# Fanchuana/OPUS-PLLM

Measured on AMD Instinct MI355X. Metric: proteins_per_sec, higher is better.
Workload: dtype f16; 1 GPU; OPUS-PLLM-llama3_8b shape: batch 64/GPU, 512-residue proteins, 89-id prompt (+8 protein tokens = 96 positions), 32 new tokens, greedy (BASELINE configs[3] per-GPU shard: batch 512 over 8 GPUs); batch_per_gpu=64, residues=512, parallelism=replicas x1 (batch-sharded), all-gather of ids

## Files before the change

### include/opus_pllm.h

```cpp
#ifndef OPUS_PLLM_H
#define OPUS_PLLM_H

#include <stdint.h>

#ifdef __cplusplus
extern "C" {
#endif

#define OPUS_ABI_VERSION 10

enum opus_status {
    OPUS_OK = 0,
    OPUS_EBADARG = -1,
    OPUS_ESHAPE = -2,
    OPUS_EHIP = -3,
    OPUS_ERCCL = -4,
    OPUS_EUNSUPPORTED = -5,
    OPUS_ESTATE = -6
};

enum opus_dtype { OPUS_F16 = 0, OPUS_F32 = 1, OPUS_I32 = 2, OPUS_I64 = 3, OPUS_U8 = 4, OPUS_F8E4M3 = 5, OPUS_I8 = 6,
                  OPUS_F4E2M1X2 = 7, OPUS_E8M0 = 8 };

typedef struct opus_config {
// ... 160 lines not shown
int opus_debug_argmax_lse(opus_ctx *ctx, const float *d_logits, int32_t B, int32_t V, int32_t *d_idx, float *d_lse, void *stream);
int opus_debug_guidance(opus_ctx *ctx, float *d_logits, int32_t P, int32_t V, float guidance_scale, void *stream);

int opus_set_logits_processors(opus_ctx *ctx, float repetition_penalty, int32_t no_repeat_ngram_size, int32_t min_new_tokens,
                               const int32_t *bad_ids, const int32_t *bad_offsets, int32_t n_bad);
int opus_debug_logits_process(opus_ctx *ctx, float *d_logits, int32_t B, int32_t V, const int32_t *d_hist, int32_t hist_stride,
                              int32_t hist_len, const int32_t *eos_ids, int32_t n_eos, float repetition_penalty,
                              int32_t no_repeat_ngram_size, int32_t min_new_tokens, const int32_t *bad_ids,
                              const int32_t *bad_offsets, int32_t n_bad, void *stream);

int opus_set_token_constraint(opus_ctx *ctx, int32_t n_states, const int32_t *edge_off, const int32_t *edge_tok,
                              const int32_t *edge_next, int32_t n_edges, const uint8_t *completing, const int32_t *end_ids,
                              int32_t n_end, const int32_t *start, int32_t n_start, void *stream);
int opus_debug_token_constraint(opus_ctx *ctx, float *d_logits, int32_t B, int32_t V, const int32_t *d_hist, int32_t hist_stride,
                                int32_t hist_len, int32_t *d_state_out, void *stream);

int opus_debug_gemm(opus_ctx *ctx, const void *d_A, const void *d_W, const float *d_bias, const float *d_residual,
                    void *d_C, int32_t M, int32_t N, int32_t K, int32_t epi, int32_t out_f32, void *stream);
int opus_debug_gemm_norm(opus_ctx *ctx, const float *d_A, const void *d_W, void *d_C, int32_t M, int32_t N, int32_t K,
                         int32_t epi, int32_t out_f32, float eps, void *stream);
int opus_debug_gemm_slabs(opus_ctx *ctx, const void *d_A, const void *d_W, float *d_slabs, int32_t M, int32_t N, int32_t K,
                          int32_t *ks, void *stream);
int opus_debug_gemm_plan(opus_ctx *ctx, int32_t *plan);
int opus_debug_gemm_w8(opus_ctx *ctx, int32_t form, const void *d_A, const void *d_W, const void *d_q8, const void *d_e8,
                       const float *d_bias, const float *d_residual, void *d_C, int32_t M, int32_t N, int32_t K, int32_t epi,
                       int32_t out_f32, float eps, int32_t *ks, int32_t *ran_w8, void *stream);
int opus_debug_gemm_w4(opus_ctx *ctx, int32_t form, const void *d_A, const void *d_W, const void *d_q4, const void *d_s4,
                       const float *d_bias, const float *d_residual, void *d_C, int32_t M, int32_t N, int32_t K, int32_t epi,
                       int32_t out_f32, float eps, int32_t *ks, int32_t *ran_w4, void *stream);
int opus_debug_knob(opus_ctx *ctx, const char *name, int32_t value);
int opus_debug_gemm_rowscale(opus_ctx *ctx, const void *d_A, const void *d_W1, float *d_X, const void *d_W2, void *d_C,
                             int32_t M, int32_t N1, int32_t K1, int32_t N2, int32_t epi, float eps, int32_t *fused,
                             void *stream);
int opus_debug_gemm_rope(opus_ctx *ctx, const void *d_A, const void *d_W, const float *d_bias, void *d_out, int32_t M,
                         int32_t D, int32_t K, int32_t T, int32_t heads, int32_t allow_fuse, int32_t *fused, void *stream);
int opus_debug_gemm_ln(opus_ctx *ctx, const void *d_A, const void *d_W1, const float *d_b1, float *d_X, float *d_part, void *d_xh,
                       float *d_stat, const void *d_W2, const float *d_c2, const float *d_colsum, void *d_C, int32_t M, int32_t N1,
                       int32_t K1, int32_t N2, int32_t epi, int32_t rms, float eps, int32_t rope_T, const int32_t *d_rope_pos,
                       int32_t *produced, int32_t *plan, void *stream);
int opus_debug_attention(opus_ctx *ctx, const void *d_Q, const void *d_K, const void *d_V, void *d_O,
                         const int32_t *d_kstart, const int32_t *d_kend, int32_t B, int32_t T, int32_t heads,
                         int32_t group, int32_t head_dim, int32_t causal, float scale, void *stream);

int opus_debug_attn_prefill(opus_ctx *ctx, const void *d_Q, const void *d_K, const void *d_V, void *d_O, int64_t q_st, int64_t k_st,
                            int64_t v_st, int64_t o_st, int64_t q_sb, int64_t k_sb, int64_t v_sb, int64_t o_sb,
                            const int32_t *d_kstart, const int32_t *d_kend, const int32_t *d_cu, int32_t B, int32_t T,
                            int32_t heads, int32_t group, int32_t head_dim, int32_t causal, int32_t q_trim, float scale,
                            int32_t *qt_used, void *stream);

int opus_debug_attn_decode(opus_ctx *ctx, const void *d_qkv, const void *d_k_hist, const void *d_v_hist, const int32_t *d_kstart,
                           int32_t B, int32_t T0, int32_t step, void *d_out, void *d_k_new, void *d_v_new, void *stream);

int opus_debug_attn_decode_form(opus_ctx *ctx, const void *d_qkv, const float *d_slabs, int32_t ks, const float *d_row_ssq,
                                int32_t row_nblk, int32_t K, float eps, const float *d_bias, const void *d_k_hist,
                                const void *d_v_hist, const int32_t *d_kstart, int32_t B, int32_t T0, int32_t step,
                                int32_t out_tiled, void *d_out, void *d_k_new, void *d_v_new, void *d_k_cache, void *d_v_cache,
                                int32_t *gp_used, void *stream);

int opus_check_error(opus_ctx *ctx, void *stream);

int opus_beam_topk(opus_ctx *ctx, const float *d_run_scores, int32_t B, int32_t K, int32_t M, float *d_scores, int32_t *d_idx,
                   void *stream);
int opus_kv_reorder(opus_ctx *ctx, const int32_t *d_src_rows, int32_t R, void *stream);
int opus_beam_sample_topk(opus_ctx *ctx, const float *d_logits, const float *d_run_scores, int32_t B, int32_t K, int32_t M,
                          float temperature, float top_p, uint64_t seed, int32_t step, float *d_scores, int32_t *d_idx, void *stream);
int opus_set_sampling_top_k(opus_ctx *ctx, int32_t k);
// ... 27 lines not shown
```

### opus-pllm_amd/_cabi.py

```python
from __future__ import annotations

import ctypes as C
import os
from typing import Optional

from .config import OpusConfig

_HERE = os.path.dirname(os.path.abspath(__file__))
BF16 = os.environ.get("OPUS_DTYPE", "fp16").lower() in ("bf16", "bfloat16")
LIB_PATH = os.environ.get("OPUS_LIB_PATH") or os.path.join(_HERE, "lib", "libopus_pllm_bf16.so" if BF16 else "libopus_pllm.so")
ABI_VERSION = 10

OPUS_F16, OPUS_F32, OPUS_I32, OPUS_I64, OPUS_U8 = 0, 1, 2, 3, 4
OPUS_F8E4M3, OPUS_I8 = 5, 6
OPUS_F4E2M1X2, OPUS_E8M0 = 7, 8


def operand_dtype():
    import torch
    return torch.bfloat16 if BF16 else torch.float16


class OpusError(RuntimeError):
    def __init__(self, code: int, msg: str):
# ... 123 lines not shown
    "opus_llama_score_tree": (C.c_int, [_P, _P, C.c_int32, _P, _P, _P, C.c_int32, _P, C.c_int32, _P, _P, _P, C.c_int32, _P, _P, _P,
                                        C.c_int32, _P, C.c_int32, _P, _P, C.c_int32, C.c_int64, _P, _P, C.c_int64, _P, C.c_int64, _P]),
    "opus_llama_score_tree_scratch_bytes": (C.c_int64, [C.POINTER(CConfig), C.c_int32, C.c_int32, C.c_int32, C.c_int32, C.c_int32,
                                                        C.c_int32]),
    "opus_llama_dec_rows_cap": (C.c_int64, [C.POINTER(CConfig)]),
    "opus_llama_tree_max_depth": (C.c_int32, []),
    "opus_trie_path_sums": (C.c_int, [_P, _P, _P, _P, _P, _P, C.c_int32, C.c_int32, C.c_int32, _P, _P]),
    "opus_debug_attn_tree": (C.c_int, [_P, _P, _P, _P, _P, C.c_int32, C.c_int32, C.c_int32, _P, _P, _P, _P, _P]),
    "opus_debug_xent": (C.c_int, [_P, _P, C.c_int32, C.c_int32, _P, _P, _P, _P]),
    "opus_esm2_contacts_packed": (C.c_int, [_P, _P, C.POINTER(C.c_int32), C.c_int32, _P, _P, _P, C.c_int64, _P]),
    "opus_esm2_contacts_scratch_bytes": (C.c_int64, [C.POINTER(CConfig), C.POINTER(C.c_int32), C.c_int32]),
    "opus_debug_contacts": (C.c_int, [_P, _P, _P, C.c_int64, C.POINTER(C.c_int32), C.c_int32, C.c_int32, C.c_int32, _P, _P, _P, _P,
                                      _P, C.c_int64, _P]),
    "opus_esm2_lm_head": (C.c_int, [_P, _P, C.c_int32, C.c_int32, _P, _P]),
    "opus_debug_esm2_lm_head": (C.c_int, [_P, _P, C.c_int32, C.c_int32, _P, _P]),
    "opus_generate_scored": (C.c_int, [_P, _P, _P, C.c_int32, C.c_int32, C.c_int32, C.POINTER(C.c_int32), C.c_int32, C.c_int32,
                                       C.c_float, C.c_float, C.c_uint64, _P, C.POINTER(C.c_int32), _P, _P, _P, _P]),
    "opus_llama_prefill_fanout": (C.c_int, [_P, _P, _P, C.c_int32, C.c_int32, C.c_int32, _P, _P]),
    "opus_generate_scored_fanout": (C.c_int, [_P, _P, _P, C.c_int32, C.c_int32, C.c_int32, C.c_int32, C.POINTER(C.c_int32), C.c_int32,
                                              C.c_int32, C.c_float, C.c_float, C.c_uint64, _P, C.POINTER(C.c_int32), _P, _P, _P, _P]),
    "opus_debug_argmax_lse": (C.c_int, [_P, _P, C.c_int32, C.c_int32, _P, _P, _P]),
    "opus_generate_scored_guided": (C.c_int, [_P, _P, _P, C.c_int32, C.c_int32, C.c_float, C.c_int32, C.POINTER(C.c_int32), C.c_int32,
                                              C.c_int32, C.c_float, C.c_float, C.c_uint64, _P, C.POINTER(C.c_int32), _P, _P, _P, _P]),
    "opus_debug_guidance": (C.c_int, [_P, _P, C.c_int32, C.c_int32, C.c_float, _P]),
    "opus_set_logits_processors": (C.c_int, [_P, C.c_float, C.c_int32, C.c_int32, C.POINTER(C.c_int32), C.POINTER(C.c_int32),
                                             C.c_int32]),
    "opus_debug_logits_process": (C.c_int, [_P, _P, C.c_int32, C.c_int32, _P, C.c_int32, C.c_int32, C.POINTER(C.c_int32), C.c_int32,
                                            C.c_float, C.c_int32, C.c_int32, C.POINTER(C.c_int32), C.POINTER(C.c_int32), C.c_int32,
                                            _P]),
    "opus_set_token_constraint": (C.c_int, [_P, C.c_int32, _P, _P, _P, C.c_int32, _P, _P, C.c_int32, _P, C.c_int32, _P]),
    "opus_debug_token_constraint": (C.c_int, [_P, _P, C.c_int32, C.c_int32, _P, C.c_int32, C.c_int32, _P, _P]),
    "opus_debug_gemm_rowscale": (C.c_int, [_P, _P, _P, _P, _P, _P, C.c_int32, C.c_int32, C.c_int32, C.c_int32, C.c_int32,
                                           C.c_float, C.POINTER(C.c_int32), _P]),
    "opus_debug_gemm_ln": (C.c_int, [_P, _P, _P, _P, _P, _P, _P, _P, _P, _P, _P, _P, C.c_int32, C.c_int32, C.c_int32, C.c_int32,
                                     C.c_int32, C.c_int32, C.c_float, C.c_int32, _P, C.POINTER(C.c_int32), C.POINTER(C.c_int32), _P]),
}

_lib: Optional[C.CDLL] = None


def lib() -> C.CDLL:
    global _lib
    if _lib is not None:
        return _lib
    if not os.path.exists(LIB_PATH):
        raise OpusError(-100, f"{LIB_PATH} not found: build it with `python opus-pllm_amd/build.py` "
                              "(hipcc --offload-arch=gfx950); this package has no CPU fallback")
    l = C.CDLL(LIB_PATH)
    for name, (res, args) in SIGNATURES.items():
        fn = getattr(l, name)
        fn.restype = res
        fn.argtypes = args
    v = l.opus_abi_version()
    if v != ABI_VERSION:
        raise OpusError(-101, f"ABI version mismatch: library {v}, binding {ABI_VERSION}")
    if l.opus_operand_dtype() != (1 if BF16 else 0):
        raise OpusError(-102, f"{LIB_PATH} was not built for {'bf16' if BF16 else 'fp16'} operands")
    _lib = l
    return l


def check(code: int) -> None:
    if code != 0:
        raise OpusError(code, lib().opus_last_error().decode("utf-8", "replace"))
```

### opus-pllm_amd/csrc/api.cpp

```cpp
#include "../../include/opus_pllm.h"
#include "common.h"

#include <cmath>
#include <cstdarg>
#include <cstdio>
#include <cstdlib>
#include <cstring>
#include <algorithm>
#include <atomic>
#include <map>
#include <string>
#include <vector>

using namespace opus;

static thread_local char g_err[512] = "";
static int fail(int code, const char *fmt, ...) {
    va_list ap;
    va_start(ap, fmt);
    vsnprintf(g_err, sizeof(g_err), fmt, ap);
    va_end(ap);
    return code;
}
#define HIPC(expr)                                                                                   \
// ... 3181 lines not shown
    const int hd = D / heads;
    if (hd != c->cfg.enc_dim / c->cfg.enc_heads || T > c->cfg.max_enc_tokens)
        return fail(OPUS_ESHAPE, "debug_gemm_rope: head_dim / T must match the context's encoder rotary table");
    HIPC(hipSetDevice(c->device));
    hipStream_t s = (hipStream_t)stream;
    const float qs = 1.0f / sqrtf((float)hd);
    GemmGot got;
    OPC(gemm(c, s, (const half_t *)A, K, (const half_t *)W, M, 3 * D, K, bias, EPI_NONE, nullptr, out, 3 * D, 0,
             GemmAsk().rope(allow_fuse && hd == 64 ? c->cs_enc : nullptr, nullptr, T, D, qs), &got));
    *fused = got.rope_done;
    if (!got.rope_done) HIPC(launch_esm_rope((half_t *)out, c->cs_enc, M / T, T, heads, hd, qs, s));
    return OPUS_OK;
}

extern "C" int opus_debug_gemm_rowscale(opus_ctx *c, const void *A, const void *W1, float *X, const void *W2, void *Cp, int32_t M,
                                        int32_t N1, int32_t K1, int32_t N2, int32_t epi, float eps, int32_t *fused, void *stream) {
    if (!c || !A || !W1 || !X || !W2 || !Cp || !fused) return fail(OPUS_EBADARG, "debug_gemm_rowscale: null pointer");
    if (M < 1 || N1 < 64 || N1 % 64 || K1 < 64 || K1 % 64 || N2 < 32) return fail(OPUS_ESHAPE, "debug_gemm_rowscale: shape");
    if (epi != EPI_NONE && epi != EPI_SILU_GU16) return fail(OPUS_EBADARG, "debug_gemm_rowscale: epilogue 0 or 2");
    const opus_config &g = c->cfg;
    if ((int64_t)M * N1 > (int64_t)g.max_batch * g.max_prompt * g.dec_dim) return fail(OPUS_ESHAPE, "debug_gemm_rowscale: M * N1 exceeds the scratch");
    HIPC(hipSetDevice(c->device));
    hipStream_t s = (hipStream_t)stream;
    ResidShadow sh;
    GemmGot got;
    OPC(gemm(c, s, (const half_t *)A, K1, (const half_t *)W1, M, N1, K1, nullptr, EPI_NONE, X, X, N1, 1,
             GemmAsk().copy16(fuse_rows() && M <= 96 ? c->d_xn : nullptr), &got));
    sh.produced(X, got);
    *fused = sh.xh_src != nullptr && (N1 & 255) == 0 && gemm_goes_wide(M, N2) ? 1 : 0;
    const int nout = epi == EPI_SILU_GU16 ? N2 / 2 : N2;
    return gemm_norm(c, s, sh, X, eps, c->d_xn, (const half_t *)W2, M, N2, N1, epi, Cp, nout, 0);
}

extern "C" int opus_debug_gemm_ln(opus_ctx *c, const void *A, const void *W1, const float *b1, float *X, float *part, void *xh,
                                  float *stat, const void *W2, const float *c2, const float *colsum, void *Cp, int32_t M, int32_t N1,
                                  int32_t K1, int32_t N2, int32_t epi, int32_t rms, float eps, int32_t rope_T,
                                  const int32_t *rope_pos, int32_t *produced, int32_t *plan, void *stream) {
    if (!c || !A || !W1 || !X || !part || !xh || !stat || !W2 || !Cp || !produced || !plan)
        return fail(OPUS_EBADARG, "debug_gemm_ln: null pointer");
    if (M < 1 || N1 < 64 || N1 % 64 || K1 < 64 || K1 % 64 || N2 < 32) return fail(OPUS_ESHAPE, "debug_gemm_ln: shape");
    if (epi != EPI_NONE && epi != EPI_GELU && epi != EPI_SILU_GU16) return fail(OPUS_EBADARG, "debug_gemm_ln: epilogue 0, 1 or 2");
    if (epi == EPI_SILU_GU16 && (!rms || c2 || colsum || N2 % 32))
        return fail(OPUS_EBADARG, "debug_gemm_ln: the gate / up epilogue is the RMSNorm form (no bias, no column sums)");
    if (rms ? colsum != nullptr : colsum == nullptr) return fail(OPUS_EBADARG, "debug_gemm_ln: column sums go with LayerNorm only");
    if (rope_pos && rope_T < 1) return fail(OPUS_EBADARG, "debug_gemm_ln: rope_pos needs rope_T");
    if (rope_T > 0 && (epi != EPI_NONE || N2 % 3 || (N2 / 3) % 64 || c->cfg.enc_dim / c->cfg.enc_heads != 64 ||
                       rope_T > c->cfg.max_enc_tokens))
        return fail(OPUS_ESHAPE, "debug_gemm_ln: rotary needs EPI_NONE, N2 = 3 D, head_dim 64 and rope_T within the context's table");
    HIPC(hipSetDevice(c->device));
    hipStream_t s = (hipStream_t)stream;
    c->phase = PH_OTHER;
    for (int i = 0; i < 2 * PP_PLAN_WORDS; ++i) plan[i] = -1;
    HIPC(hipMemsetAsync(c->d_cnt, 0, HANDOFF_ERR * sizeof(int32_t), s));
    GemmGot got;
    OPC(gemm(c, s, (const half_t *)A, K1, (const half_t *)W1, M, N1, K1, b1, EPI_NONE, X, X, N1, 1,
             GemmAsk().ln_produce(gemm_goes_pp(M, N1) ? part : nullptr, (half_t *)xh).report_pp(plan), &got));
    *produced = got.ln_done;
    if (!got.ln_done) return OPUS_OK;
    KL(KC_NORM, 8.0 * M * (N1 / 64), launch_ln_finalize(part, M, N1 / 64, N1, eps, rms, stat, s));
    const int nout = epi == EPI_SILU_GU16 ? N2 / 2 : N2;
    OPC(gemm(c, s, (const half_t *)xh, N1, (const half_t *)W2, M, N2, N1, c2, epi, nullptr, Cp, nout, 0,
             GemmAsk().ln_consume(stat, colsum).report_pp(plan + PP_PLAN_WORDS)
                 .rope(rope_T > 0 ? c->cs_enc : nullptr, rope_pos, rope_T, N2 / 3, 0.125f), &got));
    if (rope_T > 0 && !got.rope_done) return fail(OPUS_ESTATE, "debug_gemm_ln: the consumer GEMM did not fuse the rotary");
    return OPUS_OK;
}
// ... 375 lines not shown
```

### opus-pllm_amd/csrc/common.h

```cpp
#pragma once
#include <hip/hip_runtime.h>
#include <hip/hip_ext.h>
#include <stdint.h>

namespace opus {

#ifdef OPUS_BF16
typedef __bf16 half_t;
typedef __bf16 h8 __attribute__((ext_vector_type(8)));
typedef __bf16 h4 __attribute__((ext_vector_type(4)));
typedef __bf16 h2 __attribute__((ext_vector_type(2)));
#else
typedef _Float16 half_t;
typedef _Float16 h8 __attribute__((ext_vector_type(8)));
typedef _Float16 h4 __attribute__((ext_vector_type(4)));
typedef _Float16 h2 __attribute__((ext_vector_type(2)));
#endif
typedef float f4 __attribute__((ext_vector_type(4)));
__device__ __forceinline__ f4 mfma16(h8 a, h8 b, f4 c) {
#ifdef OPUS_BF16
    return __builtin_amdgcn_mfma_f32_16x16x32_bf16(a, b, c, 0, 0, 0);
#else
    return __builtin_amdgcn_mfma_f32_16x16x32_f16(a, b, c, 0, 0, 0);
#endif
// ... 116 lines not shown
    const float *bias;
    const float *residual;
    int64_t ldr;
    void *C;
    int64_t ldc;
    int out_f32;
    int epi;
    float *ws;
    int64_t ws_bytes;
    half_t *xh_out;
    float *ssq_out;
    int *fused_done;
    const float *row_ssq;
    int row_nblk;
    int64_t ssq_cap = 0;
    int *nblk_out = nullptr;
    int slab_only = 0;
    int *ks_out = nullptr;
    int force_wide = 0;
    const float *rope_cs = nullptr;
    const int32_t *rope_pos = nullptr;
    int rope_T = 0, rope_cols = 0, rope_qcols = 0;
    float rope_qscale = 1.0f;
    int *rope_done = nullptr;
    int a_tiled = 0, xh_tiled = 0, c_tiled = 0;
    int *combine_cnt = nullptr;
    float *ln_part = nullptr;
    int *ln_done = nullptr;
    const float *ln_stat = nullptr;
    const float *ln_colsum = nullptr;
    int pp_gm = 8;
    int stagger = 0;
    int no_rot = 0;
    long long *trace = nullptr;
    int *pp_plan = nullptr;
    int *plan = nullptr;
    const uint8_t *q8 = nullptr;
    const int8_t *e8 = nullptr;
    int *ran_w8 = nullptr;
    const uint8_t *q4 = nullptr;
    const uint8_t *s4 = nullptr;
    int *ran_w4 = nullptr;
};
constexpr int PP_PLAN_WORDS = 5;
enum PpTail { PP_TAIL_NONE = 0, PP_TAIL_PAIR = 1, PP_TAIL_REDUCE = 2 };
constexpr int GEMM_PLAN_WORDS = 8;
enum GemmCombine { GC_NONE = 0, GC_REDUCE = 1, GC_REDUCE4 = 2, GC_IN_LAUNCH = 3, GC_PP_PAIR = 4, GC_PP_REDUCE = 5, GC_SLABS = 6 };
inline void gemm_plan_set(const GemmParams &p, int klass, int mt, int tn, int ns, int alds, int P, int ks, int combine) {
    if (!p.plan) return;
    const int v[GEMM_PLAN_WORDS] = {klass, mt, tn, ns, alds, P, ks, combine};
    for (int i = 0; i < GEMM_PLAN_WORDS; ++i) p.plan[i] = v[i];
}

struct AttnParams {
    const half_t *Q, *K, *V;
    int64_t q_sb, q_st, k_sb, k_st, v_sb, v_st;
    half_t *O;
    int64_t o_sb, o_st;
    const int32_t *kstart;
    const int32_t *kend;
    int B, T, heads, group, head_dim, causal;
    float scale;
    const int32_t *cu = nullptr;
    int q_trim = 0;
};

// ... 3 lines not shown
bool gemm_stream_would(int M, int N, int K, int slab_only, int a_tiled, int row_scale, int64_t ws_bytes);
hipError_t launch_gemm_stream(const GemmParams &p, hipStream_t s);
struct Knobs {
    int no_stream = 0;
    int no_ln_fusion = 0;
    int debug_a_tiled = 0;
    int pp_gm = 8;
    int enc_full_last_layer = 0;
    int misc[8] = {0, 0, 0, 0, 0, 0, 0, 0};
};
extern Knobs g_knobs;
template <int NWAVES, int ROWS>
__device__ __forceinline__ void block_row_rstd(const float *__restrict__ ssq, int M, int nblk, float inv_k, float eps, float *out,
                                               int wave, int lane) {
    constexpr int RW = (ROWS + NWAVES - 1) / NWAVES;
    float part[RW];
#pragma unroll
    for (int r = 0; r < RW; ++r) part[r] = 0.f;
    for (int j0 = 0; j0 < nblk; j0 += 256) {
        float t[RW][4];
#pragma unroll
        for (int r = 0; r < RW; ++r) {
            int row = wave + NWAVES * r;
            row = row < M ? row : M - 1;
#pragma unroll
            for (int u = 0; u < 4; ++u) {
                const int j = j0 + 64 * u + lane;
                t[r][u] = ssq[(int64_t)row * nblk + (j < nblk ? j : nblk - 1)];
                t[r][u] = j < nblk ? t[r][u] : 0.f;
            }
        }
#pragma unroll
        for (int r = 0; r < RW; ++r) part[r] += (t[r][0] + t[r][1]) + (t[r][2] + t[r][3]);
    }
#pragma unroll
    for (int r = 0; r < RW; ++r) {
        float q = part[r];
#pragma unroll
        for (int o = 32; o > 0; o >>= 1) q += __shfl_xor(q, o, 64);
        const int row = wave + NWAVES * r;
        if (lane == 0 && row < ROWS) out[row] = rsqrtf(q * inv_k + eps);
    }
}
bool gemm_goes_wide(int M, int N);
bool gemm_goes_pp(int M, int N);
hipError_t launch_attn_prefill(const AttnParams &p, hipStream_t s);
int attn_prefill_query_tiles(const AttnParams &p);
struct AttnPrefixParams {
    const half_t *kc, *vc;
    int64_t cache_sb, cache_sh;
    const int32_t *kstart;
    int Tp;
    const half_t *qkv;
    int n;
    const int32_t *list, *off, *blocks;
    half_t *out;
    int nh, nkv, hd;
    float scale;
    const int32_t *par = nullptr;
};
int attn_prefix_blocks(const int32_t *off, int P, int G, int n, int32_t *blocks);
int attn_prefix_max_blocks(int R, int P, int G, int n);
hipError_t launch_attn_prefix(const AttnPrefixParams &p, int nblocks, hipStream_t s);

hipError_t launch_kv_export(const half_t *kc, const half_t *vc, int64_t cache_sl, int64_t cache_sb, int64_t cache_sh, int layers, int R,
                            int nkv, int T, int hd, half_t *snap_k, half_t *snap_v, hipStream_t s);
// ... 223 lines not shown
```

### opus-pllm_amd/csrc/gemm.hip

```cpp
#include "common.h"
#include <cstdlib>
#include <map>
#include <type_traits>
#include <mutex>
#include <utility>

namespace opus {

thread_local LaunchEvents *tl_launch_ev = nullptr;
static Knobs knobs_from_env() {
    Knobs k;
    for (int i = 0; i < 8; ++i) {
        char name[32];
        snprintf(name, sizeof(name), "OPUS_KNOB_MISC%d", i);
        if (const char *v = getenv(name)) k.misc[i] = atoi(v);
    }
    return k;
}
Knobs g_knobs = knobs_from_env();

hipError_t ensure_dyn_lds(const void *fn, size_t bytes) {
    static std::mutex mu;
    static std::map<std::pair<int, const void *>, size_t> done;
    int dev = 0;
    hipError_t e = hipGetDevice(&dev);
    if (e != hipSuccess) return e;
    std::lock_guard<std::mutex> lock(mu);
    size_t &have = done[std::make_pair(dev, fn)];
    if (bytes <= have) return hipSuccess;
    e = hipFuncSetAttribute(fn, hipFuncAttributeMaxDynamicSharedMemorySize, (int)bytes);
    if (e == hipSuccess) have = bytes;
    return e;
}

__device__ __forceinline__ float gelu_erf(float x) {
// ... 1975 lines not shown
    }
}

template <int EPI>
static hipError_t launch_reduce(const GemmParams &p, int ks, hipStream_t s) {
    const int nout = EPI == EPI_SILU_GU16 ? p.N / 2 : p.N;
    GemmParams q = p;
    if (EPI == EPI_NONE && p.xh_out && p.ssq_out && p.fused_done && p.out_f32 && !p.Af && (p.N & 255) == 0 &&
        (int64_t)p.M * (p.N >> 8) <= p.ssq_cap) {
        *p.fused_done = 1;
        if (p.nblk_out) *p.nblk_out = p.N >> 8;
    } else {
        q.xh_out = nullptr;
    }
    if (tl_launch_ev) tl_launch_ev->aux_bytes = 4.0 * ks * p.M * p.N + (double)p.M * nout * ((p.out_f32 ? 4 : 2) + (p.residual ? 4 : 0));
    const bool by4 = EPI == EPI_NONE && (p.N & 255) == 0 && ((p.ldc | p.ldr) & 3) == 0;
    if (p.plan) p.plan[7] = by4 ? GC_REDUCE4 : GC_REDUCE;
    if (by4)
        OPUS_LAUNCH(KC_REDUCE, splitk_reduce4_kernel, dim3(cdiv((int64_t)p.M * p.N, 1024)), dim3(256), 0, s, q, ks);
    else
        OPUS_LAUNCH(KC_REDUCE, (splitk_reduce_kernel<EPI>), dim3(cdiv((int64_t)p.M * nout, 256)), dim3(256), 0, s, q, ks);
    return hipGetLastError();
}

hipError_t launch_splitk_reduce(const GemmParams &p, int ks, hipStream_t s) {
    switch (p.epi) {
        case EPI_NONE: return launch_reduce<EPI_NONE>(p, ks, s);
        case EPI_GELU: return launch_reduce<EPI_GELU>(p, ks, s);
        case EPI_SILU_GU16: return launch_reduce<EPI_SILU_GU16>(p, ks, s);
    }
    return hipErrorInvalidValue;
}

template <int MT, int EPI, bool W8 = false, bool W4 = false>
__global__ __launch_bounds__(512) void gemm_wide_kernel(GemmParams p, int ksplit) {
    static_assert(!(W8 && W4), "one quantised form at a time");
    extern __shared__ __attribute__((aligned(16))) char smem[];
    OPUS_ARGS_ONE_BATCH(p);
    constexpr int MP = 16 * MT;
    constexpr int SC = MT <= 4 ? 8 : 4;
    constexpr int CIMG = MP * 128;
    constexpr int STAGE = SC * CIMG;
    constexpr int NPIECE = SC * MP / 8;
    constexpr int PW = NPIECE / 8;
    constexpr int LPC = W8 ? 1 : 2;
    const int tid = threadIdx.x, lane = tid & 63;
    const int wave = __builtin_amdgcn_readfirstlane(tid >> 6);
    const int g = lane >> 4, li = lane & 15;
    const int chunks = p.K >> 6;
    const int npanels = (p.N + 15) >> 4;
    int panel = blockIdx.x * 8 + wave;
    const bool panel_ok = panel < npanels;
    panel = panel_ok ? panel : npanels - 1;
    const int ky = blockIdx.y;
    const int c0 = kpart_begin(chunks, ky, ksplit), c1 = kpart_begin(chunks, ky + 1, ksplit);
    const half_t *wp = p.W + ((int64_t)panel * chunks) * 1024 + lane * 8;
    const uint8_t *qp = W8 ? p.q8 + ((int64_t)panel * chunks) * 1024 + lane * 16 : nullptr;
    const uint8_t *q4p = W4 ? p.q4 + ((int64_t)panel * chunks) * 512 + lane * 8 : nullptr;
    const uint8_t *s4p = W4 ? p.s4 + ((int64_t)panel * chunks) * 32 + li * 2 : nullptr;

    typedef const __attribute__((address_space(1))) void *gptr_t;
    typedef __attribute__((address_space(3))) void *lptr_t;
    int pc[PW];
    const half_t *psrc[PW];
#pragma unroll
    for (int j = 0; j < PW; ++j) {
        const int q = wave * PW + j;
        const int ch = q / (MP / 8), r = 8 * (q % (MP / 8)) + (lane >> 3);
        int row = r < p.M ? r : p.M - 1;
// ... 53 lines not shown
    };
    auto ring_load = [&](int u, int cn) {
        if constexpr (W4) ld_q4(w4q[u], w4s[u], q4p + (int64_t)cn * 512, s4p + (int64_t)cn * 32);
        else if constexpr (W8) ld_q(wq[u], qp + (int64_t)cn * 1024);
        else ld_nt(wl[u], wh[u], wp + (int64_t)cn * 1024);
    };
    auto ring_pin = [&](int u) {
        if constexpr (W4) asm volatile("" : "+v"(w4q[u]), "+v"(w4s[u]));
        else if constexpr (W8) asm volatile("" : "+v"(wq[u]));
        else asm volatile("" : "+v"(wl[u]), "+v"(wh[u]));
    };
    auto ring_mul = [&](int u, int i, h8 a0, h8 a1) {
        if constexpr (W4) {
            h8 w0, w1;
            mx4x16_to_h8(w4q[u], w4s[u], w0, w1);
            acc[i] = mfma16(w0, a0, acc[i]);
            acc[i] = mfma16(w1, a1, acc[i]);
        } else if constexpr (W8) {
            h8 w0, w1;
            fp8x16_to_h8(wq[u], w0, w1);
            acc[i] = mfma16(w0, a0, acc[i]);
            acc[i] = mfma16(w1, a1, acc[i]);
        } else {
            acc[i] = mfma16(wl[u], a0, acc[i]);
            acc[i] = mfma16(wh[u], a1, acc[i]);
        }
    };
#pragma unroll
    for (int u = 0; u < U; ++u) {
        const int cn = phys(c0 + u < c1 ? c0 + u : c1 - 1);
        ring_load(u, cn);
    }
    float *rstd_s = reinterpret_cast<float *>(smem + 2 * STAGE);
    if (p.row_ssq) block_row_rstd<8, MP>(p.row_ssq, p.M, p.row_nblk, 1.0f / (float)p.K, p.norm_eps, rstd_s, wave, lane);
    int buf = 0, cs = c0;
    auto full_stage = [&](auto has_next_tag) {
        constexpr bool HAS_NEXT = decltype(has_next_tag)::value;
        constexpr int PWN = HAS_NEXT ? PW : 0;
        asm volatile("s_waitcnt vmcnt(%0)" ::"n"(LPC * U) : "memory");
        asm volatile("s_waitcnt lgkmcnt(0)" ::: "memory");
        __builtin_amdgcn_s_barrier();
        if (HAS_NEXT) dma_stage(buf ^ 1, cs + SC);
        const char *base = smem + buf * STAGE;
        h8 fa[2][MT][2];
        auto read_chunk = [&](int u8, h8 (&f)[MT][2]) {
#pragma unroll
            for (int i = 0; i < MT; ++i) {
                f[i][0] = *reinterpret_cast<const h8 *>(base + u8 * CIMG + aoff[i]);
                f[i][1] = *reinterpret_cast<const h8 *>(base + u8 * CIMG + (aoff[i] ^ 64));
            }
        };
        read_chunk(0, fa[0]);
#pragma unroll
        for (int u8 = 0; u8 < SC; ++u8) {
            const int c = cs + u8;
            const int u = u8 & (U - 1);
            if (u8 + 1 < SC) read_chunk(u8 + 1, fa[(u8 + 1) & 1]);
            if constexpr (W4) {
                if (u8 < U) asm volatile("s_waitcnt vmcnt(%2)" : "+v"(w4q[u]), "+v"(w4s[u]) : "n"(LPC * (U - 1) + PWN));
                else asm volatile("s_waitcnt vmcnt(%2)" : "+v"(w4q[u]), "+v"(w4s[u]) : "n"(LPC * (U - 1)));
            } else if constexpr (W8) {
                if (u8 < U) asm volatile("s_waitcnt vmcnt(%1)" : "+v"(wq[u]) : "n"(LPC * (U - 1) + PWN));
                else asm volatile("s_waitcnt vmcnt(%1)" : "+v"(wq[u]) : "n"(LPC * (U - 1)));
            } else {
                if (u8 < U) asm volatile("s_waitcnt vmcnt(%2)" : "+v"(wl[u]), "+v"(wh[u]) : "n"(2 * (U - 1) + PWN));
                else asm volatile("s_waitcnt vmcnt(%2)" : "+v"(wl[u]), "+v"(wh[u]) : "n"(2 * (U - 1)));
            }
#pragma unroll
            for (int i = 0; i < MT; ++i) ring_mul(u, i, fa[u8 & 1][i][0], fa[u8 & 1][i][1]);
            const int cn = phys(c + U < c1 ? c + U : c1 - 1);
            ring_pin(u);
            ring_load(u, cn);
        }
    };
    for (; cs + SC < c1; cs += SC, buf ^= 1) full_stage(std::true_type{});
    if (cs + SC == c1) {
        full_stage(std::false_type{});
        cs += SC;
        buf ^= 1;
    }
    asm volatile("s_waitcnt vmcnt(0)" ::: "memory");
#pragma unroll
    for (int u = 0; u < U; ++u) ring_pin(u);
    if (cs < c1) {
        asm volatile("s_waitcnt lgkmcnt(0)" ::: "memory");
        __builtin_amdgcn_s_barrier();
        const char *base = smem + buf * STAGE;
#pragma unroll
        for (int u8 = 0; u8 < SC; ++u8) {
            const int c = cs + u8;
            if (c < c1) {
                const int u = u8 & (U - 1);
#pragma unroll
                for (int i = 0; i < MT; ++i) {
                    const h8 a0 = *reinterpret_cast<const h8 *>(base + u8 * CIMG + aoff[i]);
                    const h8 a1 = *reinterpret_cast<const h8 *>(base + u8 * CIMG + (aoff[i] ^ 64));
                    ring_mul(u, i, a0, a1);
                }
                w_load(u, c + U);
            }
        }
    }

    if constexpr (W8) {
        const uint32_t e4 = *reinterpret_cast<const uint32_t *>(p.e8 + panel * 16 + 4 * g);
#pragma unroll
        for (int r = 0; r < 4; ++r) {
            const float sc = exp2_i8((int)(int8_t)(e4 >> (8 * r)));
#pragma unroll
            for (int i = 0; i < MT; ++i) acc[i][r] *= sc;
        }
    }
    if (ksplit > 1) {
        float *slab = p.ws + (int64_t)ky * p.M * p.N;
        if (panel_ok) {
#pragma unroll
            for (int i = 0; i < MT; ++i) {
                const int m = 16 * i + li, nb = panel * 16 + 4 * g;
                if (m < p.M) {
#pragma unroll
                    for (int r = 0; r < 4; ++r)
                        if (nb + r < p.N) slab[(int64_t)m * p.N + nb + r] = acc[i][r];
                }
            }
        }
        return;
    }
    if (p.row_ssq) {
#pragma unroll
        for (int i = 0; i < MT; ++i) {
            const float rs = rstd_s[16 * i + li];
#pragma unroll
            for (int r = 0; r < 4; ++r) acc[i][r] *= rs;
        }
    }
    if (EPI == EPI_SILU_GU16) {
        __syncthreads();
        float *xch = reinterpret_cast<float *>(smem);
        if (wave & 1) {
#pragma unroll
            for (int i = 0; i < MT; ++i)
#pragma unroll
                for (int r = 0; r < 4; ++r) xch[(((wave >> 1) * MT + i) * 4 + r) * 64 + lane] = acc[i][r];
        }
        __syncthreads();
        if ((wave & 1) == 0 && panel_ok) {
#pragma unroll
            for (int i = 0; i < MT; ++i) {
                const int m = 16 * i + li;
                if (m >= p.M) continue;
                f4 up;
#pragma unroll
                for (int r = 0; r < 4; ++r) up[r] = xch[(((wave >> 1) * MT + i) * 4 + r) * 64 + lane];
                store4<EPI>(p, m, panel * 16 + 4 * g, acc[i], up);
            }
        }
    } else if (panel_ok) {
#pragma unroll
        for (int i = 0; i < MT; ++i) {
            const int m = 16 * i + li;
            if (m < p.M) store4<EPI>(p, m, panel * 16 + 4 * g, acc[i], acc[i]);
        }
    }
}

template <int MT, int EPI, bool W8 = false, bool W4 = false>
static hipError_t launch_wide(const GemmParams &p, hipStream_t s) {
    if constexpr (!W8 && !W4) {
        if (p.q8 && p.e8) return launch_wide<MT, EPI, true>(p, s);
        if (p.q4 && p.s4) return launch_wide<MT, EPI, false, true>(p, s);
    }
    const int blocks = cdiv((p.N + 15) >> 4, 8), chunks = p.K / 64;
    int ks = 1;
    if (p.ws && blocks < 200) {
        ks = 256 / blocks;
        ks = ks > 8 ? 8 : ks;
        if (ks > chunks / 8) ks = chunks / 8;
        while (ks > 1 && (int64_t)ks * p.M * p.N * 4 > p.ws_bytes) --ks;
        if (ks < 1) ks = 1;
    }
    if (p.ks_out) *p.ks_out = ks;
    const int lds = 2 * (MT <= 4 ? 8 : 4) * 16 * MT * 128 + 16 * MT * (int)sizeof(float);
    hipError_t ea = ensure_dyn_lds(reinterpret_cast<const void *>(&gemm_wide_kernel<MT, EPI, W8, W4>), lds);
    if (ea != hipSuccess) return ea;
    gemm_plan_set(p, KC_WIDE, MT, 0, 0, 0, 0, ks, ks == 1 ? GC_NONE : GC_SLABS);
    if (W8 && p.ran_w8) *p.ran_w8 = 1;
    if (W4 && p.ran_w4) *p.ran_w4 = 1;
    if (ks > 1 && p.row_ssq) {
        GemmParams q = p;
        q.row_ssq = nullptr;
        OPUS_LAUNCH(KC_WIDE, (gemm_wide_kernel<MT, EPI, W8, W4>), dim3(blocks, ks), dim3(512), lds, s, q, ks);
    } else {
        OPUS_LAUNCH(KC_WIDE, (gemm_wide_kernel<MT, EPI, W8, W4>), dim3(blocks, ks), dim3(512), lds, s, p, ks);
    }
    hipError_t e = hipGetLastError();
    if (e != hipSuccess || ks == 1 || p.slab_only) return e;
    return launch_reduce<EPI>(p, ks, s);
}


template <int MT, int EPI, bool NORM, bool W8 = false, bool W4 = false>
static hipError_t launch_mid_t(const GemmParams &p, hipStream_t s) {
    if constexpr (!W8 && !W4 && MT <= 4) {
        if (p.q8 && p.e8) return launch_mid_t<MT, EPI, NORM, true>(p, s);
        if (p.q4 && p.s4) return launch_mid_t<MT, EPI, NORM, false, true>(p, s);
    }
    const int blocks = cdiv((p.N + 15) >> 4, 4), chunks = p.K / 64;
    int ks = 1;
    if (p.ws && blocks < 384) {
        ks = cdiv(512, blocks);
        ks = ks > 8 ? 8 : ks;
        if (ks > chunks / 4) ks = chunks / 4;
        while (ks > 1 && ((int64_t)ks * p.M * p.N + (int64_t)ks * p.M) * 4 > p.ws_bytes) --ks;
        if (ks < 1) ks = 1;
    }
    constexpr int CH = MT <= 2 ? 4 : 1;
    const size_t lds = 2 * CH * 16 * MT * 128 + 16 * MT * sizeof(float) + 2 * MT * 4 * 64 * sizeof(float);
    if (lds > 48 * 1024) {
        hipError_t ea = ensure_dyn_lds(reinterpret_cast<const void *>(&gemm_mid_kernel<MT, EPI, NORM, W8, W4>), lds);
        if (ea != hipSuccess) return ea;
    }
    if (p.row_ssq && ks == 1) return hipErrorInvalidValue;
    gemm_plan_set(p, KC_MID, MT, 0, 0, 0, 0, ks, GC_NONE);
    if (W8 && p.ran_w8) *p.ran_w8 = 1;
    if (W4 && p.ran_w4) *p.ran_w4 = 1;
    OPUS_LAUNCH(KC_MID, (gemm_mid_kernel<MT, EPI, NORM, W8, W4>), dim3(blocks, ks), dim3(256), lds, s, p, ks);
    hipError_t e = hipGetLastError();
// ... 188 lines not shown
```

Before: 260.1 proteins/s.

## Defer wide-GEMM row-norm sum loads into final stage to overlap MFMA

In the wide GEMM kernel, the per-row RMS sum-of-squares loads used for row scaling are moved from before the main loop into the last full pipeline stage, where they are issued between MFMA chunks and awaited only at the end, with vmcnt counts adjusted to match. The prologue reduction is kept as a 'ramp' path, chosen by a knob or when the grid is large. The intent is to take the row-rstd reduction off the critical path before the first MFMA. It also adds an env-gated timing trace variant and a debug entry point for a GEMM with row sum-of-squares scaling. The hand-tuned vmcnt accounting is fragile, and the extra syncthreads in the epilogue adds a barrier.

```diff
diff --git a/include/opus_pllm.h b/include/opus_pllm.h
--- a/include/opus_pllm.h
+++ b/include/opus_pllm.h
@@ -216,6 +216,9 @@
 int opus_debug_gemm_rowscale(opus_ctx *ctx, const void *d_A, const void *d_W1, float *d_X, const void *d_W2, void *d_C,
                              int32_t M, int32_t N1, int32_t K1, int32_t N2, int32_t epi, float eps, int32_t *fused,
                              void *stream);
+int opus_debug_gemm_rowssq(opus_ctx *ctx, const void *d_A, const void *d_W, const void *d_q8, const void *d_e8, const void *d_q4,
+                           const void *d_s4, const float *d_ssq, int32_t row_nblk, float eps, void *d_C, int32_t M, int32_t N,
+                           int32_t K, int32_t epi, int32_t out_f32, void *stream);
 int opus_debug_gemm_rope(opus_ctx *ctx, const void *d_A, const void *d_W, const float *d_bias, void *d_out, int32_t M,
                          int32_t D, int32_t K, int32_t T, int32_t heads, int32_t allow_fuse, int32_t *fused, void *stream);
 int opus_debug_gemm_ln(opus_ctx *ctx, const void *d_A, const void *d_W1, const float *d_b1, float *d_X, float *d_part, void *d_xh,
diff --git a/opus-pllm_amd/_cabi.py b/opus-pllm_amd/_cabi.py
--- a/opus-pllm_amd/_cabi.py
+++ b/opus-pllm_amd/_cabi.py
@@ -179,6 +179,8 @@
     "opus_debug_token_constraint": (C.c_int, [_P, _P, C.c_int32, C.c_int32, _P, C.c_int32, C.c_int32, _P, _P]),
     "opus_debug_gemm_rowscale": (C.c_int, [_P, _P, _P, _P, _P, _P, C.c_int32, C.c_int32, C.c_int32, C.c_int32, C.c_int32,
                                            C.c_float, C.POINTER(C.c_int32), _P]),
+    "opus_debug_gemm_rowssq": (C.c_int, [_P, _P, _P, _P, _P, _P, _P, _P, C.c_int32, C.c_float, _P, C.c_int32, C.c_int32, C.c_int32,
+                                         C.c_int32, C.c_int32, _P]),
     "opus_debug_gemm_ln": (C.c_int, [_P, _P, _P, _P, _P, _P, _P, _P, _P, _P, _P, _P, C.c_int32, C.c_int32, C.c_int32, C.c_int32,
                                      C.c_int32, C.c_int32, C.c_float, C.c_int32, _P, C.POINTER(C.c_int32), C.POINTER(C.c_int32), _P]),
 }
diff --git a/opus-pllm_amd/csrc/api.cpp b/opus-pllm_amd/csrc/api.cpp
--- a/opus-pllm_amd/csrc/api.cpp
+++ b/opus-pllm_amd/csrc/api.cpp
@@ -3237,6 +3237,25 @@
     return gemm_norm(c, s, sh, X, eps, c->d_xn, (const half_t *)W2, M, N2, N1, epi, Cp, nout, 0);
 }
 
+extern "C" int opus_debug_gemm_rowssq(opus_ctx *c, const void *A, const void *W, const void *q8, const void *e8, const void *q4,
+                                      const void *s4, const float *ssq, int32_t row_nblk, float eps, void *Cp, int32_t M, int32_t N,
+                                      int32_t K, int32_t epi, int32_t out_f32, void *stream) {
+    if (!c || !A || !W || !ssq || !Cp) return fail(OPUS_EBADARG, "debug_gemm_rowssq: null pointer");
+    if (M < 1 || N < 1 || K < 64 || K % 64) return fail(OPUS_ESHAPE, "debug_gemm_rowssq: K must be a positive multiple of 64");
+    if ((epi != EPI_NONE && epi != EPI_SILU_GU16) || (epi == EPI_SILU_GU16 && N % 32)) return fail(OPUS_EBADARG, "debug_gemm_rowssq: epilogue 0 or 2");
+    if (row_nblk < 1 || (int64_t)M * row_nblk > c->ssq_cap)
+        return fail(OPUS_ESHAPE, "debug_gemm_rowssq: M * row_nblk = %lld exceeds the %lld sums the context holds", (long long)M * row_nblk, (long long)c->ssq_cap);
+    if ((q8 != nullptr) != (e8 != nullptr) || (q4 != nullptr) != (s4 != nullptr) || (q8 && q4))
+        return fail(OPUS_EBADARG, "debug_gemm_rowssq: one quantised form at most, both of its pointers");
+    if (!gemm_goes_wide(M, N)) return fail(OPUS_ESHAPE, "debug_gemm_rowssq: M=%d N=%d is not a shape of the wide kernel", M, N);
+    HIPC(hipSetDevice(c->device));
+    hipStream_t s = (hipStream_t)stream;
+    HIPC(hipMemcpyAsync(c->d_ssq, ssq, (size_t)M * row_nblk * sizeof(float), hipMemcpyDeviceToDevice, s));
+    const int nout = epi == EPI_SILU_GU16 ? N / 2 : N;
+    return gemm(c, s, (const half_t *)A, K, (const half_t *)W, M, N, K, nullptr, epi, nullptr, Cp, nout, out_f32,
+                GemmAsk().scale_rows(eps, row_nblk).w8((const uint8_t *)q8, (const int8_t *)e8).w4((const uint8_t *)q4, (const uint8_t *)s4));
+}
+
 extern "C" int opus_debug_gemm_ln(opus_ctx *c, const void *A, const void *W1, const float *b1, float *X, float *part, void *xh,
                                   float *stat, const void *W2, const float *c2, const float *colsum, void *Cp, int32_t M, int32_t N1,
                                   int32_t K1, int32_t N2, int32_t epi, int32_t rms, float eps, int32_t rope_T,
diff --git a/opus-pllm_amd/csrc/common.h b/opus-pllm_amd/csrc/common.h
--- a/opus-pllm_amd/csrc/common.h
+++ b/opus-pllm_amd/csrc/common.h
@@ -172,6 +172,7 @@
     int pp_gm = 8;
     int stagger = 0;
     int no_rot = 0;
+    int rs_ramp = 0;
     long long *trace = nullptr;
     int *pp_plan = nullptr;
     int *plan = nullptr;
@@ -241,6 +242,62 @@
         }
 #pragma unroll
         for (int r = 0; r < RW; ++r) part[r] += (t[r][0] + t[r][1]) + (t[r][2] + t[r][3]);
+    }
+#pragma unroll
+    for (int r = 0; r < RW; ++r) {
+        float q = part[r];
+#pragma unroll
+        for (int o = 32; o > 0; o >>= 1) q += __shfl_xor(q, o, 64);
+        const int row = wave + NWAVES * r;
+        if (lane == 0 && row < ROWS) out[row] = rsqrtf(q * inv_k + eps);
+    }
+}
+template <int NWAVES, int ROWS>
+__device__ __forceinline__ void row_ssq_request(const float *__restrict__ ssq, int M, int nblk, int wave, int lane,
+                                                float (&t)[(ROWS + NWAVES - 1) / NWAVES][4]) {
+    constexpr int RW = (ROWS + NWAVES - 1) / NWAVES;
+    uint32_t off[4];
+#pragma unroll
+    for (int u = 0; u < 4; ++u) {
+        const int j = 64 * u + lane;
+        off[u] = (uint32_t)(j < nblk ? j : nblk - 1) * 4u;
+    }
+#pragma unroll
+    for (int r = 0; r < RW; ++r) {
+        int row = wave + NWAVES * r;
+        row = row < M ? row : M - 1;
+        const float *base = ssq + (int64_t)row * nblk;
+#pragma unroll
+        for (int u = 0; u < 4; ++u) asm volatile("global_load_dword %0, %1, %2" : "=&v"(t[r][u]) : "v"(off[u]), "s"(base));
+    }
+}
+template <int NWAVES, int ROWS>
+__device__ __forceinline__ void row_rstd_finish(const float *__restrict__ ssq, int M, int nblk, float inv_k, float eps, float *out,
+                                                int wave, int lane, float (&t)[(ROWS + NWAVES - 1) / NWAVES][4]) {
+    constexpr int RW = (ROWS + NWAVES - 1) / NWAVES;
+    float part[RW];
+#pragma unroll
+    for (int r = 0; r < RW; ++r) {
+        part[r] = 0.f;
+#pragma unroll
+        for (int u = 0; u < 4; ++u) t[r][u] = 64 * u + lane < nblk ? t[r][u] : 0.f;
+        part[r] += (t[r][0] + t[r][1]) + (t[r][2] + t[r][3]);
+    }
+    for (int j0 = 256; j0 < nblk; j0 += 256) {
+        float v[RW][4];
+#pragma unroll
+        for (int r = 0; r < RW; ++r) {
+            int row = wave + NWAVES * r;
+            row = row < M ? row : M - 1;
+#pragma unroll
+            for (int u = 0; u < 4; ++u) {
+                const int j = j0 + 64 * u + lane;
+                v[r][u] = ssq[(int64_t)row * nblk + (j < nblk ? j : nblk - 1)];
+                v[r][u] = j < nblk ? v[r][u] : 0.f;
+            }
+        }
+#pragma unroll
+        for (int r = 0; r < RW; ++r) part[r] += (v[r][0] + v[r][1]) + (v[r][2] + v[r][3]);
     }
 #pragma unroll
     for (int r = 0; r < RW; ++r) {
diff --git a/opus-pllm_amd/csrc/gemm.hip b/opus-pllm_amd/csrc/gemm.hip
--- a/opus-pllm_amd/csrc/gemm.hip
+++ b/opus-pllm_amd/csrc/gemm.hip
@@ -1,6 +1,9 @@
 #include "common.h"
+#include <algorithm>
+#include <cstdio>
 #include <cstdlib>
 #include <map>
+#include <vector>
 #include <type_traits>
 #include <mutex>
 #include <utility>
@@ -2042,9 +2045,13 @@
     return hipErrorInvalidValue;
 }
 
-template <int MT, int EPI, bool W8 = false, bool W4 = false>
+constexpr int WIDE_TRACE_WORDS = 48, WIDE_TRACE_STAGES = 20;
+template <int MT, int EPI, bool W8 = false, bool W4 = false, bool TRACE = false>
 __global__ __launch_bounds__(512) void gemm_wide_kernel(GemmParams p, int ksplit) {
     static_assert(!(W8 && W4), "one quantised form at a time");
+    long long t_start = 0, t_mfma = 0, t_loop = 0;
+    int tstage = 0;
+    if constexpr (TRACE) t_start = wall_clock64();
     extern __shared__ __attribute__((aligned(16))) char smem[];
     OPUS_ARGS_ONE_BATCH(p);
     constexpr int MP = 16 * MT;
@@ -2164,13 +2171,27 @@
         ring_load(u, cn);
     }
     float *rstd_s = reinterpret_cast<float *>(smem + 2 * STAGE);
-    if (p.row_ssq) block_row_rstd<8, MP>(p.row_ssq, p.M, p.row_nblk, 1.0f / (float)p.K, p.norm_eps, rstd_s, wave, lane);
+    constexpr int RSW = (MP + 7) / 8;
+    constexpr int NRS = 4 * RSW;
+    float rsq[RSW][4];
+    const bool rs_late = p.row_ssq && !p.rs_ramp;
+    const float *rs_src = rs_late ? p.row_ssq : reinterpret_cast<const float *>(p.A);
+    const int rs_rows = rs_late ? p.M : 1, rs_nblk = rs_late ? p.row_nblk : 1;
+    if (p.row_ssq && p.rs_ramp) block_row_rstd<8, MP>(p.row_ssq, p.M, p.row_nblk, 1.0f / (float)p.K, p.norm_eps, rstd_s, wave, lane);
+    long long *tl = reinterpret_cast<long long *>(smem + 2 * STAGE + MP * (int)sizeof(float));
     int buf = 0, cs = c0;
     auto full_stage = [&](auto has_next_tag) {
         constexpr bool HAS_NEXT = decltype(has_next_tag)::value;
+        constexpr bool RS = !HAS_NEXT;
         constexpr int PWN = HAS_NEXT ? PW : 0;
+        constexpr int IP = SC - U - 1;
+        static_assert(LPC * (U - 1) + NRS < 64, "vmcnt range");
         asm volatile("s_waitcnt vmcnt(%0)" ::"n"(LPC * U) : "memory");
         asm volatile("s_waitcnt lgkmcnt(0)" ::: "memory");
+        if constexpr (TRACE) {
+            if (lane == 0 && tstage < WIDE_TRACE_STAGES) tl[tstage * 8 + wave] = wall_clock64();
+            ++tstage;
+        }
         __builtin_amdgcn_s_barrier();
         if (HAS_NEXT) dma_stage(buf ^ 1, cs + SC);
         const char *base = smem + buf * STAGE;
@@ -2183,30 +2204,42 @@
             }
         };
         read_chunk(0, fa[0]);
+        if constexpr (RS && IP < 0) row_ssq_request<8, MP>(rs_src, rs_rows, rs_nblk, wave, lane, rsq);
 #pragma unroll
         for (int u8 = 0; u8 < SC; ++u8) {
             const int c = cs + u8;
             const int u = u8 & (U - 1);
             if (u8 + 1 < SC) read_chunk(u8 + 1, fa[(u8 + 1) & 1]);
+            const bool behind_s = RS && u8 > IP;
             if constexpr (W4) {
-                if (u8 < U) asm volatile("s_waitcnt vmcnt(%2)" : "+v"(w4q[u]), "+v"(w4s[u]) : "n"(LPC * (U - 1) + PWN));
+                if (behind_s) asm volatile("s_waitcnt vmcnt(%2)" : "+v"(w4q[u]), "+v"(w4s[u]) : "n"(LPC * (U - 1) + NRS));
+                else if (u8 < U) asm volatile("s_waitcnt vmcnt(%2)" : "+v"(w4q[u]), "+v"(w4s[u]) : "n"(LPC * (U - 1) + PWN));
                 else asm volatile("s_waitcnt vmcnt(%2)" : "+v"(w4q[u]), "+v"(w4s[u]) : "n"(LPC * (U - 1)));
             } else if constexpr (W8) {
-                if (u8 < U) asm volatile("s_waitcnt vmcnt(%1)" : "+v"(wq[u]) : "n"(LPC * (U - 1) + PWN));
+                if (behind_s) asm volatile("s_waitcnt vmcnt(%1)" : "+v"(wq[u]) : "n"(LPC * (U - 1) + NRS));
+                else if (u8 < U) asm volatile("s_waitcnt vmcnt(%1)" : "+v"(wq[u]) : "n"(LPC * (U - 1) + PWN));
                 else asm volatile("s_waitcnt vmcnt(%1)" : "+v"(wq[u]) : "n"(LPC * (U - 1)));
             } else {
-                if (u8 < U) asm volatile("s_waitcnt vmcnt(%2)" : "+v"(wl[u]), "+v"(wh[u]) : "n"(2 * (U - 1) + PWN));
+                if (behind_s) asm volatile("s_waitcnt vmcnt(%2)" : "+v"(wl[u]), "+v"(wh[u]) : "n"(2 * (U - 1) + NRS));
+                else if (u8 < U) asm volatile("s_waitcnt vmcnt(%2)" : "+v"(wl[u]), "+v"(wh[u]) : "n"(2 * (U - 1) + PWN));
                 else asm volatile("s_waitcnt vmcnt(%2)" : "+v"(wl[u]), "+v"(wh[u]) : "n"(2 * (U - 1)));
+            }
+            if constexpr (TRACE) {
+                if (u8 == 0 && cs == c0) t_mfma = wall_clock64();
             }
 #pragma unroll
             for (int i = 0; i < MT; ++i) ring_mul(u, i, fa[u8 & 1][i][0], fa[u8 & 1][i][1]);
             const int cn = phys(c + U < c1 ? c + U : c1 - 1);
             ring_pin(u);
             ring_load(u, cn);
+            if constexpr (RS && IP >= 0) {
+                if (u8 == IP) row_ssq_request<8, MP>(rs_src, rs_rows, rs_nblk, wave, lane, rsq);
+            }
         }
     };
     for (; cs + SC < c1; cs += SC, buf ^= 1) full_stage(std::true_type{});
-    if (cs + SC == c1) {
+    const bool final_full = cs + SC == c1;
+    if (final_full) {
         full_stage(std::false_type{});
         cs += SC;
         buf ^= 1;
@@ -2214,8 +2247,26 @@
     asm volatile("s_waitcnt vmcnt(0)" ::: "memory");
 #pragma unroll
     for (int u = 0; u < U; ++u) ring_pin(u);
+    auto rs_sums = [&]() {
+#pragma unroll
+        for (int r = 0; r < RSW; ++r)
+            asm volatile("s_waitcnt vmcnt(0)" : "+v"(rsq[r][0]), "+v"(rsq[r][1]), "+v"(rsq[r][2]), "+v"(rsq[r][3]));
+        row_rstd_finish<8, MP>(p.row_ssq, p.M, p.row_nblk, 1.0f / (float)p.K, p.norm_eps, rstd_s, wave, lane, rsq);
+    };
+    if (rs_late) {
+        if (final_full) {
+            rs_sums();
+        } else {
+            row_ssq_request<8, MP>(p.row_ssq, p.M, p.row_nblk, wave, lane, rsq);
+            rs_sums();
+        }
+    }
     if (cs < c1) {
         asm volatile("s_waitcnt lgkmcnt(0)" ::: "memory");
+        if constexpr (TRACE) {
+            if (lane == 0 && tstage < WIDE_TRACE_STAGES) tl[tstage * 8 + wave] = wall_clock64();
+            ++tstage;
+        }
         __builtin_amdgcn_s_barrier();
         const char *base = smem + buf * STAGE;
 #pragma unroll
@@ -2243,6 +2294,25 @@
             for (int i = 0; i < MT; ++i) acc[i][r] *= sc;
         }
     }
+    if constexpr (TRACE) t_loop = wall_clock64();
+    auto trace_end = [&]() {
+        if constexpr (TRACE) {
+            asm volatile("s_waitcnt vmcnt(0)" ::: "memory");
+            const long long t_end = wall_clock64();
+            if (lane == 0 && p.trace) {
+                long long *tr = p.trace + ((int64_t)blockIdx.y * gridDim.x + blockIdx.x) * WIDE_TRACE_WORDS;
+                auto later = [](long long *w, long long t) { atomicMax(reinterpret_cast<unsigned long long *>(w), (unsigned long long)t); };
+                const int ns = tstage < WIDE_TRACE_STAGES ? tstage : WIDE_TRACE_STAGES;
+                later(tr + 3, t_loop);
+                later(tr + 5, t_end);
+                for (int st = 0; st < ns; ++st) later(tr + 9 + 2 * st, tl[st * 8 + wave]);
+                if (wave == 0) {
+                    tr[0] = t_start; tr[1] = t_mfma; tr[2] = t_loop; tr[4] = t_end; tr[6] = ns;
+                    for (int st = 0; st < ns; ++st) tr[8 + 2 * st] = tl[st * 8];
+                }
+            }
+        }
+    };
     if (ksplit > 1) {
         float *slab = p.ws + (int64_t)ky * p.M * p.N;
         if (panel_ok) {
@@ -2256,9 +2326,11 @@
                 }
             }
         }
+        trace_end();
         return;
     }
     if (p.row_ssq) {
+        if (rs_late) __syncthreads();
 #pragma unroll
         for (int i = 0; i < MT; ++i) {
             const float rs = rstd_s[16 * i + li];
@@ -2294,6 +2366,61 @@
             if (m < p.M) store4<EPI>(p, m, panel * 16 + 4 * g, acc[i], acc[i]);
         }
     }
+    trace_end();
+}
+
+template <int EPI>
+static void wide_trace_report(const GemmParams &p, int blocks, int ks, int lds, hipStream_t s) {
+    constexpr int MAXWG = 1024;
+    static long long *tb = nullptr;
+    const int nwg = blocks * ks;
+    const size_t bytes = (size_t)MAXWG * WIDE_TRACE_WORDS * sizeof(long long);
+    if (!tb && hipMalloc((void **)&tb, bytes) != hipSuccess) tb = nullptr;
+    if (!tb || nwg > MAXWG) return;
+    const int tlds = lds + WIDE_TRACE_STAGES * 8 * (int)sizeof(long long);
+    if (ensure_dyn_lds(reinterpret_cast<const void *>(&gemm_wide_kernel<4, EPI, false, false, true>), tlds) != hipSuccess) return;
+    GemmParams q = p;
+    q.trace = tb;
+    for (int rep = 0; rep < 3; ++rep) {
+        (void)hipMemsetAsync(tb, 0, bytes, s);
+        hipLaunchKernelGGL((gemm_wide_kernel<4, EPI, false, false, true>), dim3(blocks, ks), dim3(512), tlds, s, q, ks);
+    }
+    (void)hipStreamSynchronize(s);
+    std::vector<long long> h((size_t)nwg * WIDE_TRACE_WORDS);
+    (void)hipMemcpy(h.data(), tb, h.size() * sizeof(long long), hipMemcpyDeviceToHost);
+    long long t0 = h[0];
+    int ns = 0;
+    for (int i = 0; i < nwg; ++i) {
+        t0 = std::min(t0, h[(size_t)i * WIDE_TRACE_WORDS]);
+        ns = std::max(ns, (int)h[(size_t)i * WIDE_TRACE_WORDS + 6]);
+    }
+    auto col = [&](int word, bool own, const char *nm) {
+        std::vector<double> v;
+        for (int i = 0; i < nwg; ++i) {
+            const long long *w = &h[(size_t)i * WIDE_TRACE_WORDS];
+            if (w[word]) v.push_back((w[word] - (own ? w[0] : t0)) * 0.01);
+        }
+        if (v.empty()) return;
+        std::sort(v.begin(), v.end());
+        fprintf(stderr, "   %-44s min %7.2f  p10 %7.2f  median %7.2f  p90 %7.2f  max %7.2f us\n", nm, v.front(), v[v.size() / 10],
+                v[v.size() / 2], v[v.size() * 9 / 10], v.back());
+    };
+    fprintf(stderr, "[wide trace] M=%d N=%d K=%d epi=%d ks=%d wgs=%d row_scale=%s\n", p.M, p.N, p.K, EPI, ks, nwg,
+            !p.row_ssq ? "none" : p.rs_ramp ? "ramp" : "final stage");
+    col(0, false, "start (grid)");
+    col(1, true, "first MFMA issued (own)");
+    for (int st = 0; st < ns; ++st) {
+        char nm[64];
+        snprintf(nm, sizeof(nm), "stage %d barrier, wave 0 arrives (own)", st);
+        col(8 + 2 * st, true, nm);
+        snprintf(nm, sizeof(nm), "stage %d barrier, last wave arrives (own)", st);
+        col(9 + 2 * st, true, nm);
+    }
+    col(2, true, "main loop end, wave 0 (own)");
+    col(3, true, "main loop end, last wave (own)");
+    col(4, true, "epilogue end, wave 0 (own)");
+    col(5, true, "epilogue end, last wave (own)");
+    col(5, false, "epilogue end, last wave (grid)");
 }
 
 template <int MT, int EPI, bool W8 = false, bool W4 = false>
@@ -2318,13 +2445,14 @@
     gemm_plan_set(p, KC_WIDE, MT, 0, 0, 0, 0, ks, ks == 1 ? GC_NONE : GC_SLABS);
     if (W8 && p.ran_w8) *p.ran_w8 = 1;
     if (W4 && p.ran_w4) *p.ran_w4 = 1;
-    if (ks > 1 && p.row_ssq) {
-        GemmParams q = p;
-        q.row_ssq = nullptr;
-        OPUS_LAUNCH(KC_WIDE, (gemm_wide_kernel<MT, EPI, W8, W4>), dim3(blocks, ks), dim3(512), lds, s, q, ks);
-    } else {
-        OPUS_LAUNCH(KC_WIDE, (gemm_wide_kernel<MT, EPI, W8, W4>), dim3(blocks, ks), dim3(512), lds, s, p, ks);
-    }
+    GemmParams q = p;
+    if (ks > 1) q.row_ssq = nullptr;
+    q.rs_ramp = g_knobs.misc[1] == 1 || (g_knobs.misc[1] != 2 && blocks * ks > 256);
+    if constexpr (!W8 && !W4 && MT == 4 && EPI != EPI_GELU) {
+        static const bool trace = getenv("OPUS_WIDE_TRACE") != nullptr;
+        if (trace) wide_trace_report<EPI>(q, blocks, ks, lds, s);
+    }
+    OPUS_LAUNCH(KC_WIDE, (gemm_wide_kernel<MT, EPI, W8, W4>), dim3(blocks, ks), dim3(512), lds, s, q, ks);
     hipError_t e = hipGetLastError();
     if (e != hipSuccess || ks == 1 || p.slab_only) return e;
     return launch_reduce<EPI>(p, ks, s);
```

Result: no change. 259.9 proteins/s (median of 3 runs) (-0.1%).
